# Antymon/ppo_cpp

Hardware: AMD Instinct MI355X
Metric: PPO env-steps/s (higher is better)
Workload: dtype f32; 1 GPU; BASELINE configs[2] (cfg3): env_mock-shaped synthetic env, 4096 envs x 16 steps (B=65536), MLP [256,256], 32 minibatches x 10 epochs; n_envs_per_gpu=4096, n_steps=16, n_batch_per_gpu=65536, minibatch_rows_per_gpu=2048, parallelism=dp1, env=on-device seeded synthetic env (env_mock shape), rollout buffers resident in HBM

## Files before the change

### ppo_cpp_amd/csrc/ppo_dw2.hpp

```cpp
#pragma once
#include "ppo_kernels.hpp"

#define DW2_THREADS 512
#define DW2_SPLITS 4
#define DW2_TILES 64
#define DW2_GRID (DW2_TILES * DW2_SPLITS)
#define DW2_CH 64
#define DW2_NBUF 3
template <int KP0, int AP>
struct Dw2L {
    static constexpr int UW = KP0 > AP ? KP0 : AP;
    static constexpr int OX = 0, OY = DW2_CH * 64, OU = OY + DW2_CH * 32, OW = OU + DW2_CH * UW, BUF = OW + DW2_CH * 16;
    static constexpr int LDS_FLOATS = DW2_NBUF * BUF + 64;
};
#ifdef PPO_STAMPS
#define DW2_STAMP(i) do { if (a.stamps && threadIdx.x == 0) a.stamps[(size_t)blockIdx.x * 16 + (i)] = (i) == 15 ? __builtin_amdgcn_s_memrealtime() : __builtin_readcyclecounter(); } while (0)
#else
#define DW2_STAMP(i) do { } while (0)
#endif
#define DW2_SLOTK 8

struct SlotJob { int tower; int slot_off; int dst; int in_norm; };

struct Dw2Args {
    const float* x0g;
    const float* h1[2];
    const float* h2pi;
    const float* dy0[2];
    const float* dy1[2];
    const float* dmug;
    int n;
    float* slabs; unsigned long long slab_stride;
    unsigned* counters;
    float* grad;
    float* parts;
    int w0_off[2], w1_off[2], wmu_off;
    const SlotJob* jobs; int n_jobs, jobs_per_wg;
    const float* slots[2]; int n_rowblocks, slot_w;
    float n_local; float* beta_pow; int tail_off;
    unsigned long long* stamps;
};

__device__ __forceinline__ f32x4 dw2_ld_sc1(const float* p) {
    f32x4 v;
    asm volatile("global_load_dwordx4 %0, %1, off sc1" : "=v"(v) : "v"(p) : "memory");
    return v;
}
__device__ __forceinline__ void dw2_wait4(f32x4& a, f32x4& b, f32x4& c, f32x4& d) {
    asm volatile("s_waitcnt vmcnt(0)" : "+v"(a), "+v"(b), "+v"(c), "+v"(d) :: "memory");
}

__device__ __forceinline__ void dw2_dma(const float* src_base, unsigned lane_off, float* dst) {
    const char* src = reinterpret_cast<const char*>(src_base) + lane_off;
    const unsigned lds_addr = (unsigned)__builtin_amdgcn_readfirstlane((int)(unsigned)reinterpret_cast<size_t>((__attribute__((address_space(3))) void*)dst));
    unsigned keep;
    asm volatile("s_mov_b32 %0, m0\n\ts_mov_b32 m0, %2\n\ts_nop 0\n\tglobal_load_lds_dwordx4 %1, off\n\ts_mov_b32 m0, %0" : "=&s"(keep) : "v"(src), "s"(lds_addr) : "memory");
}

template <int UWK, int NU>
__device__ __forceinline__ void dw2_read_u(float (&u)[2][NU], const float* ubuf, int wave, int g, int c) {
#pragma unroll
    for (int ks = 0; ks < 2; ++ks) {
        const float* p = ubuf + (8 * wave + 4 * ks + g) * UWK + (UWK / 16) * c;
        if constexpr (UWK == 32) {
            const float2 t = *reinterpret_cast<const float2*>(p); u[ks][0] = t.x; u[ks][1] = t.y;
            if constexpr (NU == 4) { u[ks][2] = 0.f; u[ks][3] = 0.f; }
        }
        else { const float4 t = *reinterpret_cast<const float4*>(p); u[ks][0] = t.x; u[ks][1] = t.y; u[ks][2] = t.z; u[ks][3] = t.w; }
    }
}
template <int UWK, bool U_FIRST, int NU>
__device__ __forceinline__ void dw2_strip_mma(const float (&u)[2][NU], const float (&ww)[2], f32x4 (&sacc)[NU]) {
#pragma unroll
    for (int ks = 0; ks < 2; ++ks)
#pragma unroll
        for (int t = 0; t < UWK / 16; ++t)
            sacc[t] = U_FIRST ? __builtin_amdgcn_mfma_f32_16x16x4f32(u[ks][t], ww[ks], sacc[t], 0, 0, 0)
                              : __builtin_amdgcn_mfma_f32_16x16x4f32(ww[ks], u[ks][t], sacc[t], 0, 0, 0);
}

template <int KP0, int AP, bool PEER = false>
__device__ __forceinline__ void dw2_body(const Dw2Args& a, float* lds, const int b, const PeerDev* pp = nullptr) {
    typedef Dw2L<KP0, AP> LD;
    DW2_STAMP(15); DW2_STAMP(0);
    const int tid = threadIdx.x, lane = tid & 63, wave = uni(tid >> 6);
    const int g = lane >> 4, c = lane & 15;
    const int split = (b >> 1) & 3, tower = b & 1, tile = b >> 3;
    const int gtile = tower * 32 + tile;
    const int i0 = (tile >> 3) * 64, j0 = (tile & 7) * 32;
#ifdef DW2_NOSTRIP
    const int kind = 2;
#else
    const int kind = uni(tile < 16 ? 0 : (tower == 0 ? 1 : 2));
#endif
    const int sidx = tile & 15;
    const int uwk = kind == 0 ? KP0 : AP;
    const int jl = tid >> 5, jb = b * a.jobs_per_wg + jl;
    const bool has_job = jl < a.jobs_per_wg && jb < a.n_jobs;
    const int4 jraw = reinterpret_cast<const int4*>(a.jobs)[has_job ? jb : 0];
    const int nct = a.n / DW2_CH;
    const int cb = (split * nct) >> 2, nch = (((split + 1) * nct) >> 2) - cb;
    const size_t r0 = (size_t)cb * DW2_CH;
    const float* Xg = uni(a.h1[tower]) + r0 * 256;
    const float* Yg = uni(a.dy1[tower]) + r0 * 256;
    const float* Ug = uni(kind == 1 ? a.dmug : a.x0g) + r0 * uwk;
    const float* Wg = uni(kind == 1 ? a.h2pi : a.dy0[tower]) + r0 * 256;
    const unsigned lx = (unsigned)(((lane >> 4) * 256 + i0 + 4 * (lane & 15)) * 4);
    const unsigned ly = (unsigned)(((lane >> 3) * 256 + j0 + 4 * (lane & 7)) * 4);
    const unsigned lu = (unsigned)(lane * 16);
    const unsigned lw = (unsigned)(((lane >> 2) * 256 + 16 * sidx + 4 * (lane & 3)) * 4);
    const int np = uni(3 + (kind == 2 ? 0 : (uwk >> 5) + 1));
    auto stage_x = [&](int ch) __attribute__((always_inline)) {
        float* buf = lds + (ch % DW2_NBUF) * LD::BUF;
        const size_t rb = (size_t)ch * DW2_CH;
#pragma unroll
        for (int k = 0; k < 2; ++k) { const int j = 2 * wave + k; dw2_dma(Xg + (rb + 4 * j) * 256, lx, buf + LD::OX + j * 256); }
    };
    auto stage_rest = [&](int ch) __attribute__((always_inline)) {
        float* buf = lds + (ch % DW2_NBUF) * LD::BUF;
        const size_t rb = (size_t)ch * DW2_CH;
        dw2_dma(Yg + (rb + 8 * wave) * 256, ly, buf + LD::OY + wave * 256);
        if (kind != 2) {
            if (uwk == 32) dw2_dma(Ug + rb * 32 + wave * 256, lu, buf + LD::OU + wave * 256);
            else {
#pragma unroll
                for (int k = 0; k < 2; ++k) dw2_dma(Ug + rb * 64 + (2 * wave + k) * 256, lu, buf + LD::OU + (2 * wave + k) * 256);
            }
            if (lane < 32) dw2_dma(Wg + (rb + 8 * wave) * 256, lw, buf + LD::OW + wave * 128);
        }
    };
    auto stage = [&](int ch) __attribute__((always_inline)) { stage_x(ch); stage_rest(ch); };
    auto wait_keep_one = [&]() __attribute__((always_inline)) {
        if (np == 3) asm volatile("s_waitcnt vmcnt(3)" ::: "memory");
        else if (np == 4) asm volatile("s_waitcnt vmcnt(4)" ::: "memory");
        else if (np == 5) asm volatile("s_waitcnt vmcnt(5)" ::: "memory");
        else asm volatile("s_waitcnt vmcnt(6)" ::: "memory");
    };
    if (nch > 0) stage(0);
    if (nch > 1) stage(1);
    if (nch > 2) stage(2);
    DW2_STAMP(1);
    const int ax = (8 * wave + g) * 64 + 4 * c, by = (8 * wave + g) * 32 + 2 * c;
    const int swo = (8 * wave + g) * 16 + c;
    constexpr int NU = LD::UW / 16;
    struct Frags { float4 xa[2]; float2 yb[2]; float u[2][NU]; float ww[2]; };
    auto read_main = [&](Frags& f, int ch) __attribute__((always_inline)) {
        const float* buf = lds + (ch % DW2_NBUF) * LD::BUF;
#pragma unroll
        for (int ks = 0; ks < 2; ++ks) {
            f.xa[ks] = *reinterpret_cast<const float4*>(buf + LD::OX + ax + ks * 256);
            f.yb[ks] = *reinterpret_cast<const float2*>(buf + LD::OY + by + ks * 128);
        }
    };
    auto read_strip = [&](Frags& f, int ch) __attribute__((always_inline)) {
        const float* buf = lds + (ch % DW2_NBUF) * LD::BUF;
        if (kind != 2) {
            if (KP0 == AP || kind == 0) dw2_read_u<KP0, NU>(f.u, buf + LD::OU, wave, g, c); else dw2_read_u<AP, NU>(f.u, buf + LD::OU, wave, g, c);
#pragma unroll
            for (int ks = 0; ks < 2; ++ks) f.ww[ks] = buf[LD::OW + swo + ks * 64];
        }
    };
    auto read_frags = [&](Frags& f, int ch) __attribute__((always_inline)) { read_main(f, ch); read_strip(f, ch); };
    f32x4 acc[4][2], sacc[NU];
#pragma unroll
    for (int i = 0; i < 4; ++i) acc[i][0] = acc[i][1] = (f32x4){0.f, 0.f, 0.f, 0.f};
#pragma unroll
    for (int t = 0; t < NU; ++t) sacc[t] = (f32x4){0.f, 0.f, 0.f, 0.f};
    auto mma_main = [&](const Frags& f, int ks) __attribute__((always_inline)) {
#ifdef DW2_NOMFMA
        if (a.n < 0)
#endif
        {
            const float xv[4] = {f.xa[ks].x, f.xa[ks].y, f.xa[ks].z, f.xa[ks].w};
#pragma unroll
            for (int i = 0; i < 4; ++i) {
                acc[i][0] = __builtin_amdgcn_mfma_f32_16x16x4f32(xv[i], f.yb[ks].x, acc[i][0], 0, 0, 0);
                acc[i][1] = __builtin_amdgcn_mfma_f32_16x16x4f32(xv[i], f.yb[ks].y, acc[i][1], 0, 0, 0);
            }
        }
    };
    auto mma_strip = [&](const Frags& f) __attribute__((always_inline)) {
#ifdef DW2_NOMFMA
        if (a.n < 0) {
#endif
        if (kind == 0) dw2_strip_mma<KP0, true, NU>(f.u, f.ww, sacc);
        else if (kind == 1) dw2_strip_mma<AP, false, NU>(f.u, f.ww, sacc);
#ifdef DW2_NOMFMA
        }
#endif
    };
    if (nch > 2) wait_keep_one(); else asm volatile("s_waitcnt vmcnt(0)" ::: "memory");
    __builtin_amdgcn_s_barrier();
    Frags fa, fb;
    if (nch > 0) read_frags(fa, 0);
    float sj[DW2_SLOTK];
    auto load_slots = [&]() __attribute__((always_inline)) {
        const int ln = tid & 31;
        const float* p = (jraw.x ? a.slots[1] : a.slots[0]) + jraw.y;
#pragma unroll
        for (int k = 0; k < DW2_SLOTK; ++k) { const int rb = ln + 32 * k; sj[k] = (has_job && rb < a.n_rowblocks) ? p[(size_t)rb * a.slot_w] : 0.f; }
    };
    load_slots();
    DW2_STAMP(2);
    auto iteration = [&](int i, Frags& cur, Frags& nxt) __attribute__((always_inline)) {
#ifdef DW2_NOREAD
        const bool st = i + 3 < nch, rd = false;
#else
        const bool st = i + 3 < nch, rd = i + 1 < nch;
#endif
        mma_main(cur, 0);
        __builtin_amdgcn_sched_barrier(0);
#ifndef DW2_NODMA
        if (st) stage(i + 3);
#endif
        if (rd) read_frags(nxt, i + 1);
        __builtin_amdgcn_sched_barrier(0);
        mma_main(cur, 1);
        mma_strip(cur);
        if (i + 3 < nch) wait_keep_one(); else asm volatile("s_waitcnt vmcnt(0)" ::: "memory");
        asm volatile("s_waitcnt lgkmcnt(0)" ::: "memory");
    };
    for (int i = 0; i < nch; i += 2) {
        iteration(i, fa, fb);
        if (i + 1 < nch) iteration(i + 1, fb, fa);
    }
    DW2_STAMP(3);
    __syncthreads();
    float* park = lds;
    float* spark = lds + 8 * 2048;
    static_assert(8 * 2048 + 8 * 16 * LD::UW <= DW2_NBUF * LD::BUF, "park + strip partials fit the chunk ring");
    float* red2 = lds + DW2_NBUF * LD::BUF + 32;
    const int sn = 16 * uwk;
#pragma unroll
    for (int i = 0; i < 4; ++i)
#pragma unroll
        for (int r = 0; r < 4; ++r)
            *reinterpret_cast<float2*>(park + wave * 2048 + (4 * (4 * g + r) + i) * 32 + 2 * c) = make_float2(acc[i][0][r], acc[i][1][r]);
    if (kind == 0) {
#pragma unroll
        for (int t = 0; t < KP0 / 16; ++t)
#pragma unroll
            for (int r = 0; r < 4; ++r) spark[wave * sn + ((KP0 / 16) * (4 * g + r) + t) * 16 + c] = sacc[t][r];
    } else if (kind == 1) {
#pragma unroll
        for (int r = 0; r < 4; ++r) {
            float* dst = spark + wave * sn + (4 * g + r) * AP + (AP / 16) * c;
            if constexpr (AP == 32) *reinterpret_cast<float2*>(dst) = make_float2(sacc[0][r], sacc[1][r]);
            else *reinterpret_cast<float4*>(dst) = make_float4(sacc[0][r], sacc[1][r], sacc[2][r], sacc[3][r]);
        }
    }
    {
        float s = ((sj[0] + sj[1]) + (sj[2] + sj[3])) + ((sj[4] + sj[5]) + (sj[6] + sj[7]));
        s = half_sum_lane0(s);
        if ((tid & 31) == 0) {
            if (has_job) st_wt<PEER>(a.grad + jraw.z, s);
            red2[tid >> 5] = (has_job && jraw.w) ? s * s : 0.f;
        }
    }
    __syncthreads();
    float4 m4 = *reinterpret_cast<const float4*>(park + 4 * tid);
#pragma unroll
    for (int q = 1; q < 8; ++q) { const float4 p = *reinterpret_cast<const float4*>(park + q * 2048 + 4 * tid); m4.x += p.x; m4.y += p.y; m4.z += p.z; m4.w += p.w; }
    float4 sv = make_float4(0.f, 0.f, 0.f, 0.f);
    const bool strip_thread = kind != 2 && 4 * tid < sn;
    if (strip_thread) {
        sv = *reinterpret_cast<const float4*>(spark + 4 * tid);
#pragma unroll
        for (int w = 1; w < 8; ++w) { const float4 p = *reinterpret_cast<const float4*>(spark + w * sn + 4 * tid); sv.x += p.x; sv.y += p.y; sv.z += p.z; sv.w += p.w; }
    }
    const unsigned moff = (unsigned)(a.w1_off[tower] + (i0 + (tid >> 3)) * 256 + j0 + 4 * (tid & 7));
    unsigned soff = 0;
    if (kind == 0) soff = (unsigned)(a.w0_off[tower] + (tid >> 2) * 256 + 16 * sidx + 4 * (tid & 3));
    else if (kind == 1) soff = (unsigned)(a.wmu_off + (16 * sidx + (4 * tid) / AP) * AP + (4 * tid) % AP);
    const unsigned sslab = kind == 0 ? (unsigned)(a.w0_off[tower] + sidx * sn + 4 * tid) : soff;
    float* slab = a.slabs + (size_t)split * a.slab_stride;
    st_wt4<true>(slab + moff, m4);
    if (strip_thread) st_wt4<true>(slab + sslab, sv);
    if (tid == 0) {
        float q = 0.f;
        for (int j = 0; j < 16; ++j) q += red2[j];
        a.parts[DW2_TILES + b] = q;
    }
    if (b == 0 && tid == 64) st_wt<PEER>(a.grad + a.tail_off + 5, a.n_local);
    if (b == 0 && tid == 65) { a.beta_pow[0] = a.beta_pow[2]; a.beta_pow[1] = a.beta_pow[3]; }
    DW2_STAMP(4);
    asm volatile("s_waitcnt vmcnt(0)" ::: "memory");
    __syncthreads();
    DW2_STAMP(5);
    int* flag = reinterpret_cast<int*>(lds + DW2_NBUF * LD::BUF);
    if (tid == 0) {
        const unsigned old = __hip_atomic_fetch_add(a.counters + gtile, 1u, __ATOMIC_RELAXED, __HIP_MEMORY_SCOPE_AGENT);
        flag[0] = (old == DW2_SPLITS - 1) ? 1 : 0;
    }
    __syncthreads();
    DW2_STAMP(6);
    const bool fin = flag[0] != 0;
    f32x4 t4 = {0.f, 0.f, 0.f, 0.f}, u4 = t4;
    if (fin) {
        f32x4 p[DW2_SPLITS], q[DW2_SPLITS];
#pragma unroll
        for (int s = 0; s < DW2_SPLITS; ++s) {
            p[s] = dw2_ld_sc1(a.slabs + (size_t)s * a.slab_stride + moff);
            q[s] = dw2_ld_sc1(a.slabs + (size_t)s * a.slab_stride + (strip_thread ? sslab : moff));
        }
        dw2_wait4(p[0], p[1], p[2], p[3]);
        dw2_wait4(q[0], q[1], q[2], q[3]);
        t4 = p[0]; u4 = q[0];
#pragma unroll
        for (int s = 1; s < DW2_SPLITS; ++s) { t4 += p[s]; u4 += q[s]; }
        *reinterpret_cast<float4*>(a.grad + moff) = make_float4(t4[0], t4[1], t4[2], t4[3]);
        float sq = (t4[0] * t4[0] + t4[1] * t4[1]) + (t4[2] * t4[2] + t4[3] * t4[3]);
        if (strip_thread) {
            *reinterpret_cast<float4*>(a.grad + soff) = make_float4(u4[0], u4[1], u4[2], u4[3]);
            sq += (u4[0] * u4[0] + u4[1] * u4[1]) + (u4[2] * u4[2] + u4[3] * u4[3]);
        }
        sq = wave_sum_lane0(sq);
        float* red = lds + DW2_NBUF * LD::BUF + 16;
        if (lane == 0) red[wave] = sq;
        __syncthreads();
        if (tid == 0) {
            float s = 0.f;
#pragma unroll
            for (int w = 0; w < 8; ++w) s += red[w];
            a.parts[gtile] = s;
            __hip_atomic_store(a.counters + gtile, 0u, __ATOMIC_RELAXED, __HIP_MEMORY_SCOPE_AGENT);
        }
        __syncthreads();
        if constexpr (PEER) {
            const PeerDev& p = *pp;
            const unsigned sq = __hip_atomic_load(p.seq, __ATOMIC_RELAXED, __HIP_MEMORY_SCOPE_AGENT) + 1u, par = sq & 1u;
            float jv = 0.f; int jdst = -1;
            if (tid < DW2_SPLITS * a.jobs_per_wg) {
                const int sp = tid / a.jobs_per_wg, jl2 = tid - sp * a.jobs_per_wg;
                const int jb2 = ((tile << 3) | (sp << 1) | tower) * a.jobs_per_wg + jl2;
                if (jb2 < a.n_jobs) { jdst = a.jobs[jb2].dst; jv = __hip_atomic_load(a.grad + jdst, __ATOMIC_RELAXED, __HIP_MEMORY_SCOPE_AGENT); }
            }
            const bool has_n = gtile == 0 && tid == 511;
            const float nloc = has_n ? __hip_atomic_load(a.grad + a.tail_off + 5, __ATOMIC_RELAXED, __HIP_MEMORY_SCOPE_AGENT) : 0.f;
#pragma unroll 1
            for (int k = 0; k < p.world; ++k) {
                const int r = (p.rank + k) % p.world;
                float* dst = p.slots[r] + ((unsigned long long)par * p.world + p.rank) * p.cap;
                asm volatile("global_store_dwordx4 %0, %1, off sc0 sc1" :: "v"(dst + moff), "v"(t4) : "memory");
                if (strip_thread) asm volatile("global_store_dwordx4 %0, %1, off sc0 sc1" :: "v"(dst + soff), "v"(u4) : "memory");
                if (jdst >= 0) __hip_atomic_store(dst + jdst, jv, __ATOMIC_RELAXED, __HIP_MEMORY_SCOPE_SYSTEM);
                if (has_n) __hip_atomic_store(dst + a.tail_off + 5, nloc, __ATOMIC_RELAXED, __HIP_MEMORY_SCOPE_SYSTEM);
            }
            asm volatile("s_waitcnt vmcnt(0)" ::: "memory");
            __syncthreads();
            if (tid == 0) flag[0] = (__hip_atomic_fetch_add(p.arrive, 1u, __ATOMIC_RELAXED, __HIP_MEMORY_SCOPE_AGENT) == DW2_TILES - 1u) ? 1 : 0;
            __syncthreads();
            if (flag[0]) {
                __builtin_amdgcn_fence(__ATOMIC_ACQ_REL, "");
                if (tid < (unsigned)p.world) peer_st_sys(p.flags[tid] + ((size_t)par * PEER_MAX_WORLD + p.rank) * PEER_FLAG_STRIDE, sq);
                if (tid == 0) {
                    __hip_atomic_store(p.arrive, 0u, __ATOMIC_RELAXED, __HIP_MEMORY_SCOPE_AGENT);
                    __hip_atomic_store(p.seq, sq, __ATOMIC_RELAXED, __HIP_MEMORY_SCOPE_AGENT);
                }
            }
        }
    }
    DW2_STAMP(7);
}

template <int KP0, int AP>
__global__ __launch_bounds__(DW2_THREADS) void weight_grad_assemble_kernel(Dw2Args a) {
    extern __shared__ __attribute__((aligned(16))) float lds[];
    warm_kernargs<sizeof(Dw2Args)>();
    dw2_body<KP0, AP>(a, lds, (int)blockIdx.x);
}

template <int KP0, int AP>
__global__ __launch_bounds__(DW2_THREADS) void weight_grad_assemble_peer_kernel(Dw2Args a, PeerDev p) {
    extern __shared__ __attribute__((aligned(16))) float lds[];
    warm_kernargs<sizeof(Dw2Args) + sizeof(PeerDev)>();
    dw2_body<KP0, AP, true>(a, lds, (int)blockIdx.x, &p);
}
```

Baseline: 5.031 million env-steps/s.

## Park wave partials in own chunk-ring slots, skip own-split slab reload

Each wave now writes its partial tile into its own X/Y/U pieces of the chunk ring rather than into a shared park area, which removes the __syncthreads before parking. The finishing block reuses its own register sums for its split instead of reloading them from the global slab. A trailing barrier is kept only on the peer path. The gain is one fewer block barrier plus a few global loads in the split-K gradient epilogue, at the risk of races if another wave is still reading its ring pieces.

```diff
diff --git a/ppo_cpp_amd/csrc/ppo_dw2.hpp b/ppo_cpp_amd/csrc/ppo_dw2.hpp
--- a/ppo_cpp_amd/csrc/ppo_dw2.hpp
+++ b/ppo_cpp_amd/csrc/ppo_dw2.hpp
@@ -225,26 +225,28 @@
         if (i + 1 < nch) iteration(i + 1, fb, fa);
     }
     DW2_STAMP(3);
-    __syncthreads();
-    float* park = lds;
-    float* spark = lds + 8 * 2048;
-    static_assert(8 * 2048 + 8 * 16 * LD::UW <= DW2_NBUF * LD::BUF, "park + strip partials fit the chunk ring");
+    static_assert(3 * 512 + 2 * 256 >= 2048, "a wave's own X and Y pieces hold its partial of the tile");
+    auto main_at = [&](int q, int p) __attribute__((always_inline)) {
+        return p < 1536 ? (p >> 9) * LD::BUF + LD::OX + 512 * q + (p & 511) : ((p - 1536) >> 8) * LD::BUF + LD::OY + 256 * q + ((p - 1536) & 255);
+    };
+    const int se = 8 * uwk;
+    auto strip_at = [&](int q, int sp) __attribute__((always_inline)) { return (sp / se) * LD::BUF + LD::OU + se * q + sp % se; };
     float* red2 = lds + DW2_NBUF * LD::BUF + 32;
     const int sn = 16 * uwk;
 #pragma unroll
     for (int i = 0; i < 4; ++i)
 #pragma unroll
         for (int r = 0; r < 4; ++r)
-            *reinterpret_cast<float2*>(park + wave * 2048 + (4 * (4 * g + r) + i) * 32 + 2 * c) = make_float2(acc[i][0][r], acc[i][1][r]);
+            *reinterpret_cast<float2*>(lds + main_at(wave, (4 * (4 * g + r) + i) * 32 + 2 * c)) = make_float2(acc[i][0][r], acc[i][1][r]);
     if (kind == 0) {
 #pragma unroll
         for (int t = 0; t < KP0 / 16; ++t)
 #pragma unroll
-            for (int r = 0; r < 4; ++r) spark[wave * sn + ((KP0 / 16) * (4 * g + r) + t) * 16 + c] = sacc[t][r];
+            for (int r = 0; r < 4; ++r) lds[strip_at(wave, ((KP0 / 16) * (4 * g + r) + t) * 16 + c)] = sacc[t][r];
     } else if (kind == 1) {
 #pragma unroll
         for (int r = 0; r < 4; ++r) {
-            float* dst = spark + wave * sn + (4 * g + r) * AP + (AP / 16) * c;
+            float* dst = lds + strip_at(wave, (4 * g + r) * AP + (AP / 16) * c);
             if constexpr (AP == 32) *reinterpret_cast<float2*>(dst) = make_float2(sacc[0][r], sacc[1][r]);
             else *reinterpret_cast<float4*>(dst) = make_float4(sacc[0][r], sacc[1][r], sacc[2][r], sacc[3][r]);
         }
@@ -258,15 +260,16 @@
         }
     }
     __syncthreads();
-    float4 m4 = *reinterpret_cast<const float4*>(park + 4 * tid);
-#pragma unroll
-    for (int q = 1; q < 8; ++q) { const float4 p = *reinterpret_cast<const float4*>(park + q * 2048 + 4 * tid); m4.x += p.x; m4.y += p.y; m4.z += p.z; m4.w += p.w; }
+    DW2_STAMP(8);
+    float4 m4 = *reinterpret_cast<const float4*>(lds + main_at(0, 4 * tid));
+#pragma unroll
+    for (int q = 1; q < 8; ++q) { const float4 p = *reinterpret_cast<const float4*>(lds + main_at(q, 4 * tid)); m4.x += p.x; m4.y += p.y; m4.z += p.z; m4.w += p.w; }
     float4 sv = make_float4(0.f, 0.f, 0.f, 0.f);
     const bool strip_thread = kind != 2 && 4 * tid < sn;
     if (strip_thread) {
-        sv = *reinterpret_cast<const float4*>(spark + 4 * tid);
-#pragma unroll
-        for (int w = 1; w < 8; ++w) { const float4 p = *reinterpret_cast<const float4*>(spark + w * sn + 4 * tid); sv.x += p.x; sv.y += p.y; sv.z += p.z; sv.w += p.w; }
+        sv = *reinterpret_cast<const float4*>(lds + strip_at(0, 4 * tid));
+#pragma unroll
+        for (int w = 1; w < 8; ++w) { const float4 p = *reinterpret_cast<const float4*>(lds + strip_at(w, 4 * tid)); sv.x += p.x; sv.y += p.y; sv.z += p.z; sv.w += p.w; }
     }
     const unsigned moff = (unsigned)(a.w1_off[tower] + (i0 + (tid >> 3)) * 256 + j0 + 4 * (tid & 7));
     unsigned soff = 0;
@@ -300,11 +303,15 @@
         f32x4 p[DW2_SPLITS], q[DW2_SPLITS];
 #pragma unroll
         for (int s = 0; s < DW2_SPLITS; ++s) {
-            p[s] = dw2_ld_sc1(a.slabs + (size_t)s * a.slab_stride + moff);
-            q[s] = dw2_ld_sc1(a.slabs + (size_t)s * a.slab_stride + (strip_thread ? sslab : moff));
+            p[s] = (f32x4){m4.x, m4.y, m4.z, m4.w}; q[s] = (f32x4){sv.x, sv.y, sv.z, sv.w};
+            if (s != split) {
+                p[s] = dw2_ld_sc1(a.slabs + (size_t)s * a.slab_stride + moff);
+                if (strip_thread) q[s] = dw2_ld_sc1(a.slabs + (size_t)s * a.slab_stride + sslab);
+            }
         }
         dw2_wait4(p[0], p[1], p[2], p[3]);
         dw2_wait4(q[0], q[1], q[2], q[3]);
+        DW2_STAMP(9);
         t4 = p[0]; u4 = q[0];
 #pragma unroll
         for (int s = 1; s < DW2_SPLITS; ++s) { t4 += p[s]; u4 += q[s]; }
@@ -314,6 +321,7 @@
             *reinterpret_cast<float4*>(a.grad + soff) = make_float4(u4[0], u4[1], u4[2], u4[3]);
             sq += (u4[0] * u4[0] + u4[1] * u4[1]) + (u4[2] * u4[2] + u4[3] * u4[3]);
         }
+        DW2_STAMP(10);
         sq = wave_sum_lane0(sq);
         float* red = lds + DW2_NBUF * LD::BUF + 16;
         if (lane == 0) red[wave] = sq;
@@ -325,7 +333,7 @@
             a.parts[gtile] = s;
             __hip_atomic_store(a.counters + gtile, 0u, __ATOMIC_RELAXED, __HIP_MEMORY_SCOPE_AGENT);
         }
-        __syncthreads();
+        if constexpr (PEER) __syncthreads();
         if constexpr (PEER) {
             const PeerDev& p = *pp;
             const unsigned sq = __hip_atomic_load(p.seq, __ATOMIC_RELAXED, __HIP_MEMORY_SCOPE_AGENT) + 1u, par = sq & 1u;
```

After: 5.059 million env-steps/s, median of 6. Within noise of the previous version (+0.6%).
